# acerbilab/vbmc

Measured on AMD Instinct MI355X. Metric: ELBO+grad evals/sec (Ns=1e4, K=50, D=10, N=400), higher is better.
Workload: dtype f64; 1 GPU; BASELINE configs[2]: D=10 N=400 K=50 Ns=10000/component S=20, R=64 restarts batched per GPU per step, value+gradient, beta=0, no variance; restarts_per_gpu=64, parallelism=one GPU

## Files before the change

### vbmc_amd/csrc/abi_elbo.hip

```cpp
#include <algorithm>
#include <cmath>
#include <mutex>

#include "elbo_kernels.h"
#include "var_kernels.h"
#include "gp_kernels.h"
#include <cstdlib>

extern "C" int vbmc_abi_version(void) { return VBMC_ABI_VERSION; }

static vbmc_status ctx_create_impl(int device, void* stream, vbmc_ctx** out, bool with_aux) {
  if (!out) return VBMC_ERR_INVALID;
  *out = nullptr;
  {
    static std::once_flag hq_once;
    std::call_once(hq_once, [] {
      const char* hq = getenv("VBMC_HW_QUEUES");
      if (!(hq && !strcmp(hq, "0"))) (void)setenv("GPU_MAX_HW_QUEUES", hq && atoi(hq) > 0 ? hq : "8", 0);
    });
  }
  int ndev = 0;
  if (hipGetDeviceCount(&ndev) != hipSuccess || ndev <= 0) return VBMC_ERR_NO_DEVICE;
  if (device < 0 || device >= ndev) return VBMC_ERR_NO_DEVICE;
  hipDeviceProp_t prop;
// ... 846 lines not shown
        const size_t mom_lds = LJ_MFMA_DYN_LDS(DT, nw);
        ElboDims dml = dm;
        dml.S = sh.mode == 1 ? perS : S;
        const double* al = gp->alpha + (size_t)s0 * dm.N;
        const double* gc = gp->gpc + (size_t)s0 * GPC_STRIDE(D);
        if (ns <= 0) {
        } else if (lj_mfma && mom_lds + LJ_MFMA_STATIC_LDS <= 64 * 1024) {
          if (P.compute_grad)
            hipLaunchKernelGGL((k_logjoint_mfma<DT, true>), dim3(ns, R), dim3(WAVE * nw), mom_lds, ls, dml, P.d_vpd,
                               gp->X, gp->d_meanX, al, gc, P.d_delta2, lj_out);
          else
            hipLaunchKernelGGL((k_logjoint_mfma<DT, false>), dim3(ns, R), dim3(WAVE * nw), mom_lds, ls, dml, P.d_vpd,
                               gp->X, gp->d_meanX, al, gc, P.d_delta2, lj_out);
          LAUNCH_CHECK(ctx, "k_logjoint_mfma");
          ctx->last_lj_form = P.compute_grad ? VBMC_LJFORM_MFMA_GRAD : VBMC_LJFORM_MFMA_VALUE;
        } else {
          ctx->last_lj_form = lj_split ? VBMC_LJFORM_VALU_SPLIT : VBMC_LJFORM_VALU_WAVE;
          hipLaunchKernelGGL((k_logjoint<DT>), dim3((K + 3) / 4, ns, R), dim3(lj_split ? WAVE * LJ_MAXW : WAVE), 0, ls, dml, P.d_vpd, gp->X, al, gc,
                             P.d_delta2, lj_out, P.compute_grad);
          LAUNCH_CHECK(ctx, "k_logjoint");
        }
      });
    }
    if (ctx->profiling) HIP_TRY(ctx, hipEventRecord(ctx->ev[1], ls));
    if (sh.mode == 0 && (fork || !P.mc)) hipLaunchKernelGGL(k_lj_reduce, dim3(K, R), dim3(64), 0, ls, S, K, 2 * D + 2, P.d_lj, P.d_ljbar);
    LAUNCH_CHECK(ctx, "k_lj_reduce");
    return VBMC_OK;
  };
  if (fork) {
    HIP_TRY(ctx, hipEventRecord(ctx->ev_fork, st));
    HIP_TRY(ctx, hipStreamWaitEvent(ctx->aux, ctx->ev_fork, 0));
  } else if (sh.mode != 2) {
    vbmc_status s_ = enqueue_logjoint(st);
    if (s_) return s_;
  }
  if (sh.mode == 2) {
    const size_t blk = shard_doubles(P, sh.world), ljn = shard_lj_doubles(P, sh.world);
    const size_t tot = (size_t)R * S * K * (2 * D + 2) + (P.mc ? (size_t)R * K * P.C * P.ncol : 0);
    hipLaunchKernelGGL(k_shard_scatter, dim3((unsigned)std::min<size_t>((tot + 255) / 256, 4096)), dim3(256), 0, st, R, S, K, 2 * D + 2,
                       P.C, P.ncol, sh.world, perS, perC, blk, ljn, sh.gathered, P.d_lj, P.mc ? P.d_part : nullptr);
    LAUNCH_CHECK(ctx, "k_shard_scatter");
    if (!P.mc) hipLaunchKernelGGL(k_lj_reduce, dim3(K, R), dim3(64), 0, st, S, K, 2 * D + 2, P.d_lj, P.d_ljbar);
  }

  FinArgs fa{};
  fa.dm = dm;
  if (P.mc) {
    EntArgs ea{};
    ea.entp = P.d_entp; ea.vpd = P.d_vpd;
    ea.part = sh.mode == 1 ? sh.send + shard_lj_doubles(P, sh.world) : P.d_part;
    ea.D = D; ea.K = K; ea.Mh = P.Mh; ea.C = sh.mode == 1 ? perC : P.C; ea.c0 = c0; ea.tiles_per_chunk = P.tpc; ea.ncol = P.ncol; ea.seed = seed;
    ea.eps = P.d_eps; ea.eps_stride_r = P.eps_stride_r; ea.cutoff = P.cutoff; ea.r0 = P.r0; ea.rstride = P.rstride;
    ea.prio = 1;
    ea.co_c1 = P.co_c1; ea.co_c2 = P.co_c2; ea.co_tpc2 = P.co_tpc2;
    const bool walk = P.walk_tpw > 0;
    if (walk && (sh.mode != 0 || co)) return set_err(ctx, VBMC_ERR_INVALID, "internal: the walking entropy launch was planned for a sharded / role-carrying pass");
    if (walk) { ea.walk_tpw = P.walk_tpw; ea.walk_R = R; }
    int co_rows = 0;
    if (co) {
      LjCo& lc = ea.lj;
      lc.nsplit = lj_co_nsplit(ctx, P);
      lc.nwg = ((K + 3) / 4) * S * lc.nsplit;
      if (P.use_lane) {
        lc.rows = co_rows = 0;
      } else {
        const int gx = P.co_c2 > 0 ? P.co_c1 : nc;
        lc.rows = co_rows = (std::max(lc.nwg, P.co_c2 > 0 ? K * P.co_c2 : 0) + gx - 1) / gx;
      }
      lc.want_grad = P.compute_grad;
      lc.dm = dm; lc.X = gp->X; lc.alpha = gp->alpha; lc.gpc = gp->gpc; lc.delta2 = P.d_delta2; lc.lj = P.d_lj;
    }
    if (ctx->profiling) HIP_TRY(ctx, hipEventRecord(ctx->ev[2], st));
    if (sh.mode != 2 && nc > 0) {
      ctx->last_ent_form = P.use_lane ? VBMC_ENTFORM_LANE : (P.use_mfma ? VBMC_ENTFORM_MFMA : VBMC_ENTFORM_VALU);
      if (co) ctx->last_lj_form = P.use_lane ? VBMC_LJFORM_ROLE_LANE : VBMC_LJFORM_ROLE_MFMA;
    }
    if (sh.mode == 2 || nc <= 0) {
    } else if (P.use_lane) {
      ea.nc_launch = nc;
      int gx = (K * nc + ENT_LANE_WAVES_HOST - 1) / ENT_LANE_WAVES_HOST;
      if (co) gx = std::max(gx, (ea.lj.nwg + ENT_LANE_WAVES_HOST - 1) / ENT_LANE_WAVES_HOST);
      bool ok = launch_entropy_lane(D, K, P.compute_grad != 0, dim3(gx, 1 + co_rows, R), st, ea);
      if (!ok) return set_err(ctx, VBMC_ERR_UNSUPPORTED, "no lane entropy kernel for D = %d, K = %d", D, K);
    } else if (P.use_mfma) {
      bool ok = launch_entropy_mfma(P.qs, P.kt, P.hv, P.compute_grad != 0, walk ? dim3(P.walk_nw, 1, 1) : dim3((co && P.co_c2 > 0) ? P.co_c1 : nc, K + co_rows, R), st, ea);
      if (!ok) return set_err(ctx, VBMC_ERR_UNSUPPORTED, "no MFMA entropy kernel for D = %d", D);
    } else {
      const size_t lds = P.ent_lds;
      DISPATCH_DT(dt, {
        HIP_TRY(ctx, set_entropy_lds<DT>(P.compute_grad != 0, lds));
        launch_entropy<DT>(P.compute_grad != 0, dim3(nc, K, R), lds, st, ea);
      });
    }
    LAUNCH_CHECK(ctx, "the entropy kernel");
    if (ctx->profiling) HIP_TRY(ctx, hipEventRecord(ctx->ev[3], st));
    if (sh.mode == 1) return VBMC_OK;
    if (fork)
      hipLaunchKernelGGL(k_ent_reduce, dim3(K, R), dim3(P.ncol >= 192 ? 256 : (P.ncol >= 96 ? 128 : 64)), 0, st, P.C, P.ncol,
                         P.d_part, P.d_red, P.walk_tpw, (P.Mh + 15) / 16);
    else
      hipLaunchKernelGGL(k_reduce_both, dim3(K, R, 2), dim3(P.ncol >= 192 ? 256 : (P.ncol >= 96 ? 128 : 64)), 0, st, P.C, P.ncol,
                         P.d_part, P.d_red, co ? S * ea.lj.nsplit : S, 2 * D + 2, P.d_lj, P.d_ljbar, P.walk_tpw, (P.Mh + 15) / 16);
    LAUNCH_CHECK(ctx, "k_ent_reduce / k_reduce_both");
    fa.entpart = P.d_red; fa.entlb = nullptr; fa.M = P.Mh; fa.C = 1; fa.ncol = P.ncol;
  } else {
    if (sh.mode == 1) return VBMC_OK;
// ... 723 lines not shown
```

### vbmc_amd/csrc/elbo_types.h

```cpp
#pragma once
#include <hip/hip_runtime.h>

#define WAVE 64

struct VpLayout {
  int D, K;
  __host__ __device__ int mu() const { return 0; }
  __host__ __device__ int sigma() const { return D * K; }
  __host__ __device__ int lambda() const { return D * K + K; }
  __host__ __device__ int w() const { return D * K + K + D; }
  __host__ __device__ int eta() const { return D * K + 2 * K + D; }
  __host__ __device__ int lognf() const { return D * K + 3 * K + D; }
  __host__ __device__ int lnsigma() const { return D * K + 3 * K + D + 1; }
  __host__ __device__ int lnlambda() const { return D * K + 4 * K + D + 1; }
  __host__ __device__ int stride() const { return D * K + 4 * K + 2 * D + 2; }
};
#define ENTP_EXTRA 4
#define GPC_STRIDE(D) (3 * (D) + 2)
#define OUT_HDR 5

struct ElboDims {
  int D, K, R, S, N, T;
  int opt[4];
  int off_mu, off_sigma, off_lambda, off_eta;
};


#define LJ_CO_SPLIT 8
struct LjCo {
  int rows;
  int nwg;
  int nsplit, want_grad;
  ElboDims dm;
  const double *X, *alpha, *gpc, *delta2;
  double* lj;
};

struct EntArgs {
  const double* entp;
  const double* vpd;
  const double* eps;
  long long eps_stride_r;
  double* part;
  int D, K, Mh, C, tiles_per_chunk, ncol;
  int c0;
  int prio;
  unsigned long long seed;
  int r0, rstride;
  double cutoff;
  int nc_launch;
  int co_c1, co_c2, co_tpc2;
  int walk_tpw, walk_R;
  LjCo lj;
};

__host__ __device__ inline int ent_walk_first(long long p, int ntile, int tpw) { return (int)((p * ntile) / tpw); }
__host__ __device__ inline int ent_walk_slots(long long p, int ntile, int tpw) {
  return (int)((p * ntile + ntile - 1) / tpw) - ent_walk_first(p, ntile, tpw) + 1;
}
__host__ __device__ inline int ent_walk_max_slots(int ntile, int tpw) { return (ntile - 1) / tpw + 2; }

#define VB_SMALL_PRIO() __builtin_amdgcn_s_setprio(3)
```

### vbmc_amd/csrc/entropy_mfma.h

```cpp
#pragma once
#include <type_traits>

#include "device_math.h"
#include "elbo_types.h"
#include "exp2_tab1k.h"
#include "logjoint_body.h"

typedef double mf4 __attribute__((ext_vector_type(4)));
struct EntTileAny { static constexpr bool rt = false, val = true; };
struct EntTileFull { static constexpr bool rt = false, val = false; };
struct EntTilePartial { static constexpr bool rt = false, val = true; };
#define VBMC_ENT_SPLIT(KT_, QS_, TL_, HV_) ((HV_) == 1)

#ifdef VBMC_INSTRUMENT
#define VBMC_DBG_WAVES 32768
__device__ unsigned long long g_ent_dbg[6 * VBMC_DBG_WAVES];
#endif

#define VBMC_STAG_FOR(KT_, QS_, TL_) ((KT_) == 1 || (KT_) == 4 || ((KT_) == 2 && (QS_) >= 6) || ((KT_) == 3 && (QS_) <= ((TL_) ? 5 : 8)))



constexpr bool ent_c2_for(int KT, int QS, int TL, int HV) {
  if (HV == 1) {
// ... 9 lines not shown
  }
  if (KT == 2) return !((TL == 1 && QS >= 6) || (TL == 2 && QS >= 5));
  if (KT == 3) return !(TL == 1 && QS == 7);
  return QS != 5;
}
constexpr bool ent_gp2_for(int KT, int QS, int TL, int HV) { return !(HV == 1 && KT == 1 && TL == 0 && QS <= 3); }

template <int HV>
__device__ __forceinline__ void ent_sync() {
  __builtin_amdgcn_fence(__ATOMIC_RELEASE, "wavefront");
  __builtin_amdgcn_wave_barrier();
  __builtin_amdgcn_fence(__ATOMIC_ACQUIRE, "wavefront");
}
template <int HV>
__device__ __forceinline__ void ent_sync_wg() {
  if (HV == 1) ent_sync<1>();
  else __syncthreads();
}

template <int QS, int KT, bool GRAD, bool SPARSE, int HV = 1, int TL = 0, bool CO = false, bool EM = true, bool WALK = false>
#define VBMC_ENT_EO(HV_) true
#define VBMC_ENT_ONE_WAVE(KT_, QS_, TL_, HV_) \
  (((HV_) == 1 && (KT_) == 4 && (QS_) >= 5) || ((HV_) == 1 && (KT_) == 3 && (QS_) >= 8) || ((HV_) == 4 && (KT_) == 4 && (QS_) >= 6) || \
   ((HV_) == 4 && (KT_) == 3 && (QS_) >= 9))
#define VBMC_ENT_WAVES(KT_, QS_, TL_, HV_) \
  (VBMC_ENT_ONE_WAVE(KT_, QS_, TL_, HV_) ? 1 : ((((KT_) <= 2 && (QS_) <= 4) && !((KT_) == 2 && (TL_) == 2 && (HV_) == 1)) ? 3 : 2))
__device__ __forceinline__ void ent_mfma_segment(const EntArgs& a, const int c, const int j, const int r, const int t0, const int t1,
                                                 const int pdone, const int ptot) {
  static_assert(!CO || (HV == 1 && QS <= 8 && !SPARSE), "the log-joint role exists for single-wave dense kernels at D <= 30");
  static_assert(!WALK || (HV == 1 && !CO), "the walk exists for single-wave workgroups without the log-joint role");
  static_assert(KT <= 4 && (HV == 1 || HV == 2 || HV == 4 || HV == 8), "larger mixtures are split over the waves of a workgroup (HV = 2, 4; round 5: 8, K <= 512)");
  static_assert(TL == 0 || ((TL == 1 || TL == 2) && !SPARSE), "the component tail (one or two values per lane) exists for the dense kernels only");
  constexpr int TLN = TL > 0 ? TL : 1;
  constexpr bool SP = SPARSE;
  constexpr int DP = 4 * QS;
  constexpr int NPV = (4 * QS + 15) / 16;
  constexpr int QL = QS;
  __shared__ double Et[16 * DP];
  constexpr bool GP2 = GRAD && ent_gp2_for(KT, QS, TL, HV);
  __shared__ double RQ_all[HV][GP2 ? 32 : 16];
  __shared__ double BND_all[HV][SPARSE ? KT * 16 * 3 : 1];
  constexpr int YXN = NPV * 4 * WAVE;
  constexpr bool EO = VBMC_ENT_EO(HV);
  constexpr bool YXSB = HV > 1 && EO;
  constexpr bool US = EO;
  constexpr bool VBL = GRAD && HV == 1 && (KT >= 3 || NPV >= 2);
  __shared__ double VBS_all[HV][VBL ? KT * 4 * NPV * WAVE : 1];
  constexpr bool C2 = EO && !SPARSE && ent_c2_for(KT, QS, TL, HV);
#define ENT_CI(kt_, rr_) (16 * (kt_) + 4 * (rr_) + lg)
  __shared__ __attribute__((aligned(16))) double SCP_all[HV][C2 ? KT * 16 * 2 : 2];
  __shared__ double BTL_all[HV][TL ? 4 * TL * DP : 1];
  constexpr bool NML = HV > 1 && EO;
  __shared__ double NMS_all[HV][NML ? KT * 4 * WAVE : 1];
#ifdef VBMC_INSTRUMENT
  const unsigned long long wckE = wall_clock64();
#endif
  int tid_ = threadIdx.x;
  if (WALK) asm volatile("" : "+v"(tid_));
  const int tid = tid_, wv = tid >> 6, hv = HV == 1 ? 0 : wv, lane = tid & 63;
  const int li = lane & 15, lg = lane >> 4;
  int D_ = a.D, K_ = a.K;
  const double *entp_ = a.entp, *vpd_ = a.vpd;
  double* part_ = a.part;
  if (WALK) asm volatile("" : "+s"(D_), "+s"(K_), "+s"(entp_), "+s"(vpd_), "+s"(part_));
  const int D = D_, K = K_;
  double* RQ = RQ_all[wv];
  double* NMS = NMS_all[wv];
  double* BND = BND_all[hv];
  double* VBS = VBS_all[hv];
  double* BTL = BTL_all[hv];
  double* SCP = SCP_all[hv];
  const int Kh = (K + HV - 1) / HV;
  const int kbase = hv * Kh;
  const int Kw = min(K, kbase + Kh) - kbase;
  const int PSg = D + ENTP_EXTRA;
  extern __shared__ double PB[];
  double* const TAB = PB;
  double* const YX = PB + VB_EXP_TAB1K_N;
  constexpr int NTH0 = WAVE * HV;
  constexpr int NTB0 = (VB_EXP_TAB1K_N + NTH0 - 1) / NTH0;
  double tt[NTB0];
#pragma unroll
  for (int u = 0; u < NTB0; ++u) tt[u] = c_exp2_tab1k[min(tid + u * NTH0, VB_EXP_TAB1K_N - 1)];
  const double sigj = vpd_[(size_t)r * VpLayout{D, K}.stride() + VpLayout{D, K}.sigma() + j];
  {
    const double* gsrc = entp_ + (size_t)r * K * PSg;
    constexpr int NT = WAVE * HV;
    const int n = K * PSg;
    int idx = tid;
    for (; idx + 7 * NT < n; idx += 8 * NT) {
      double t8[8];
#pragma unroll
      for (int u = 0; u < 8; ++u) t8[u] = gsrc[idx + u * NT];
#pragma unroll
      for (int u = 0; u < 8; ++u) PB[idx + u * NT] = t8[u];
    }
    {
      double t8[8];
#pragma unroll
      for (int u = 0; u < 8; ++u) t8[u] = (idx + u * NT < n) ? gsrc[idx + u * NT] : 0.0;
#pragma unroll
      for (int u = 0; u < 8; ++u) if (idx + u * NT < n) PB[idx + u * NT] = t8[u];
    }
  }
  __syncthreads();
  const double* gp = PB;
  const double* pj = gp + (size_t)j * PSg;
  const double cKj = pj[D + 1];
  const double hj_neg = 0.5 / (sigj * sigj);
  const int nr_last = TL ? 4 : max(1, min(4, (Kw - 16 * (KT - 1) + 3) >> 2));
  constexpr unsigned FULL_MASK = (1u << KT) - 1u;
  const double logwj = SPARSE ? log(pj[D + 2]) : 0.0;

  constexpr double ESC = VB_EXP_TAB1K_SCALE;
  double SA[KT][QL];
  double SC[KT];
  double VB[VBL ? 1 : KT][4][NPV];
  double WF[KT][4];
#pragma unroll
  for (int kt = 0; kt < KT; ++kt) {
    const int k = 16 * kt + li;
    const bool kv = k < Kw;
    const double* pk = gp + (size_t)(kv ? kbase + k : 0) * PSg;
    double h = pk[D];
    double m2 = 0.0;
    for (int d = 0; d < D; ++d) { double t = pk[d] - pj[d]; m2 = fma(t, t, m2); }
    if (SPARSE && lg == 0) {
      BND[(16 * kt + li) * 3 + 0] = sqrt(m2);
      BND[(16 * kt + li) * 3 + 1] = kv ? pk[D + 1] - cKj : -1.0e30;
      BND[(16 * kt + li) * 3 + 2] = h;
    }
#pragma unroll
    for (int q = 0; q < QL; ++q) {
      const int cc = 4 * q + lg;
      if (EO) {
        double sav = (kv && cc < D) ? ESC * (-2.0 * h * (pk[cc] - pj[cc])) : 0.0;
        if (C2) {
          if (cc == D) sav = kv ? ESC * (h + hj_neg) : 0.0;
          if (cc == D + 1) sav = ESC * (kv ? fma(h, m2, pk[D + 1]) - cKj : -1.0e6);
        }
        SA[kt][q] = sav;
      } else {
        double v;
        if (!kv) v = (cc == D + 1) ? -1.0e6 : 0.0;
        else if (cc < D) v = -2.0 * h * (pk[cc] - pj[cc]);
        else if (cc == D) v = h + hj_neg;
        else if (cc == D + 1) v = fma(h, m2, pk[D + 1]) - cKj;
        else v = 0.0;
        SA[kt][q] = ESC * v;
      }
    }
    SC[kt] = ESC * (!kv ? (lg == 1 ? -1.0e6 : 0.0)
                        : (lg == 0 ? h + hj_neg : (lg == 1 ? fma(h, m2, pk[D + 1]) - cKj : 0.0)));
    if (C2 && lg < 2) SCP[(16 * kt + li) * 2 + lg] = 2.0 * SC[kt];
#pragma unroll
    for (int rr = 0; rr < 4; ++rr) {
      const int k2 = ENT_CI(kt, rr);
      const bool kv2 = k2 < Kw;
      const double* p2 = gp + (size_t)(kv2 ? kbase + k2 : 0) * PSg;
      if (GRAD) {
#pragma unroll
        for (int pv = 0; pv < NPV; ++pv) {
          const int col = 16 * pv + li;
          double v = 0.0;
          if (kv2) {
            if (col == 0) v = p2[D + 2];
            else if (col == 1) v = p2[D + 3];
            else if (col < 2 + D) v = p2[D + 3] * (p2[col - 2] - pj[col - 2]);
          }
          if (VBL) VBS[((kt * 4 + rr) * NPV + pv) * WAVE + lane] = v;
          else VB[VBL ? 0 : kt][rr][pv] = v;
        }
      } else {
        WF[kt][rr] = kv2 ? p2[D + 2] : 0.0;
      }
    }
  }

  double tC0[TLN], tC1[TLN], VBt[TLN][NPV], WFt[TLN], Wt[TLN];
#pragma unroll
  for (int u = 0; u < TLN; ++u) {
    tC0[u] = 0.0; tC1[u] = 0.0; WFt[u] = 0.0; Wt[u] = 0.0;
#pragma unroll
    for (int pv = 0; pv < NPV; ++pv) VBt[u][pv] = 0.0;
  }
  if (TL) {
#pragma unroll
    for (int u = 0; u < TLN; ++u) {
      const int tq = 4 * u + lg;
      const int kq = 16 * KT + tq;
      const bool kvq = kq < Kw;
      const double* pq = gp + (size_t)(kvq ? kbase + kq : 0) * PSg;
      const double h = pq[D];
      double m2 = 0.0;
      for (int d = 0; d < D; ++d) { double t = pq[d] - pj[d]; m2 = fma(t, t, m2); }
      tC0[u] = kvq ? ESC * (h + hj_neg) : 0.0;
      tC1[u] = ESC * (kvq ? fma(h, m2, pq[D + 1]) - cKj : -1.0e6);
      for (int d = li; d < DP; d += 16) BTL[tq * DP + d] = (kvq && d < D) ? ESC * (-2.0 * h * (pq[d] - pj[d])) : 0.0;
      if (GRAD) {
#pragma unroll
        for (int pv = 0; pv < NPV; ++pv) {
          const int col = 16 * pv + li;
          double v = 0.0;
          if (kvq) {
            if (col == 0) v = pq[D + 2];
            else if (col == 1) v = pq[D + 3];
            else if (col < 2 + D) v = pq[D + 3] * (pq[col - 2] - pj[col - 2]);
          }
          VBt[u][pv] = v;
        }
      } else {
        WFt[u] = kvq ? pq[D + 2] : 0.0;
      }
    }
  }

  __syncthreads();
  {
#pragma unroll
    for (int u = 0; u < NTB0; ++u) if (VB_EXP_TAB1K_N % NTH0 == 0 || tid + u * NTH0 < VB_EXP_TAB1K_N) TAB[tid + u * NTH0] = tt[u];
  }
  __syncthreads();

#define SAV(kt_, q_) SA[kt_][q_]
  constexpr int VBR = (VBL && NPV == 1 && HV == 1 && KT == 3 && !CO) ? ((EM && QS <= 4) ? (TL == 2 ? 4 : 10) : 12) : 0;
  double VBreg[VBR > 0 ? VBR : 1];
#pragma unroll
  for (int u = 0; u < VBR; ++u) VBreg[u] = VBS[u * WAVE + lane];
#define VBV(kt_, rr_, pv_) (VBL ? (((kt_) * 4 + (rr_)) * NPV + (pv_) < VBR ? VBreg[(((kt_) * 4 + (rr_)) * NPV + (pv_)) < VBR ? (((kt_) * 4 + (rr_)) * NPV + (pv_)) : 0] : VBS[(((kt_) * 4 + (rr_)) * NPV + (pv_)) * WAVE + lane]) : VB[VBL ? 0 : (kt_)][rr_][pv_])
  double accH = 0.0, accG[NPV], accLG[NPV];
  double pm = 1.0;
  int pe = 0, pcnt = 0;
  double Wacc[KT][4];
#pragma unroll
  for (int pv = 0; pv < NPV; ++pv) { accG[pv] = 0.0; accLG[pv] = 0.0; }
#pragma unroll
  for (int kt = 0; kt < KT; ++kt)
#pragma unroll
    for (int rr = 0; rr < 4; ++rr) Wacc[kt][rr] = 0.0;

#ifdef VBMC_INSTRUMENT
  const unsigned long long wck0 = wall_clock64();
#endif
  const int ntile = (a.Mh + 15) >> 4;
  const double sfm0 = lg == 0 ? 1.0 : 0.0, sfm1 = lg == 1 ? 1.0 : 0.0;
  const int emask = (4 * (QS - 1) + lg < D) ? -1 : 0;
  const int emask2 = (QS >= 2 && 4 * (QS - 2) + lg < D) ? -1 : 0;
  const double* epsr = a.eps ? a.eps + (size_t)r * a.eps_stride_r + (size_t)j * a.Mh * D : nullptr;
  constexpr bool EPF = EM && HV == 1 && QS <= 4 && KT <= 3 && !SPARSE;
  double epre[EPF ? QS : 1];
  auto eps_fetch = [&](const int tile) {
#pragma unroll
    for (int u = 0; u < (EPF ? QS : 0); ++u) {
      const int idx = lane + u * WAVE, i = idx / DP, d = idx - i * DP;
      double v = 0.0;
      if (tile < t1 && d < D && tile * 16 + i < a.Mh) v = epsr[(size_t)(tile * 16 + i) * D + d];
      epre[u] = v;
    }
  };
  if (EPF && epsr) eps_fetch(t0);
  if (!epsr && (HV == 1 || hv == 0))
    for (int idx = lane; idx < 16 * DP; idx += WAVE) Et[idx] = 0.0;
  const int evm1 = emask, evm2 = emask2;
  const double c2u1 = (4 * (QS - 1) + lg == D) ? 1.0 : 0.0, c2o1 = (4 * (QS - 1) + lg == D + 1) ? 1.0 : 0.0;
  const double c2u2 = (QS >= 2 && 4 * (QS - 2) + lg == D) ? 1.0 : 0.0;

  auto tile_body = [&](const int tile, auto pkind) __attribute__((always_inline)) {
    using PK = decltype(pkind);
    const int b0 = tile * 16;
    ent_sync_wg<HV>();
    if (HV > 1 && hv != 0) {
    } else if (EPF && epsr) {
#pragma unroll
      for (int u = 0; u < (EPF ? QS : 0); ++u) Et[lane + u * WAVE] = US ? sigj * epre[u] : epre[u];
      eps_fetch(tile + 1);
    } else if (epsr) {
      for (int idx = lane; idx < 16 * DP; idx += WAVE) {
        const int i = idx / DP, d = idx - i * DP;
        Et[idx] = (d < D && b0 + i < a.Mh) ? (US ? sigj * epsr[(size_t)(b0 + i) * D + d] : epsr[(size_t)(b0 + i) * D + d]) : 0.0;
      }
    } else {
      unsigned long long seed_t = a.seed;
      if (WALK) asm volatile("" : "+s"(seed_t));
#pragma unroll
      for (int q = lg; q < QS; q += 4) {
        double z4[4] = {0.0, 0.0, 0.0, 0.0};
#define VBMC_RNG_CALL_FOR(KT_, QS_, TL_, HV_) ((HV_) == 2 && (((KT_) == 2 && (TL_) == 2 && (QS_) == 5) || ((KT_) == 3 && (TL_) == 0 && (QS_) == 7)))
        if constexpr (!VBMC_RNG_CALL_FOR(KT, QS, TL, HV)) {
        if (q < (D + 3) / 4) { const vb_d4 zz = vb_normal4i(seed_t, (unsigned)(b0 + li), (unsigned)j, (unsigned)(a.r0 + r * a.rstride), (unsigned)q); z4[0] = zz[0]; z4[1] = zz[1]; z4[2] = zz[2]; z4[3] = zz[3]; }
        } else {
        if (q < (D + 3) / 4) vb_normal4(seed_t, (unsigned)(b0 + li), (unsigned)j, (unsigned)(a.r0 + r * a.rstride), (unsigned)q, z4);
        }
#undef VBMC_RNG_CALL_FOR
        if (q < (D + 3) / 4) {
#pragma unroll
        for (int t = 0; t < 4; ++t) Et[li * DP + 4 * q + t] = US ? sigj * z4[t] : z4[t];
        }
      }
    }
    ent_sync_wg<HV>();
    double ev[QS];
    double e2 = 0.0;
#pragma unroll
    for (int q = 0; q < QS; ++q) {
      ev[q] = Et[li * DP + 4 * q + lg];
      if (q == QS - 1) ev[q] = __hiloint2double(__double2hiint(ev[q]) & evm1, __double2loint(ev[q]) & evm1);
      if (QS >= 2 && q == QS - 2) ev[q] = __hiloint2double(__double2hiint(ev[q]) & evm2, __double2loint(ev[q]) & evm2);
      e2 = fma(ev[q], ev[q], e2);
    }
    e2 = xor_sum16(e2);
    e2 = xor_sum32(e2);
    double shift = US ? fma(-e2, hj_neg, cKj) : cKj - 0.5 * e2;
    const double u2 = US ? e2 : sigj * sigj * e2;
    if (US && SPARSE) e2 *= 2.0 * hj_neg;
    constexpr bool partial = PK::val;
    const bool svalid = b0 + li < a.Mh;
    if (partial) shift = svalid ? shift : 0.0;
    unsigned act = FULL_MASK;
    if (SPARSE) {
      double e2m = e2;
      e2m = fmax(e2m, __shfl_xor(e2m, 1, 64)); e2m = fmax(e2m, __shfl_xor(e2m, 2, 64));
      e2m = fmax(e2m, __shfl_xor(e2m, 4, 64)); e2m = fmax(e2m, __shfl_xor(e2m, 8, 64));
      const double umax = sigj * sqrt(e2m);
      const double own = 0.5 * e2m - logwj;
      act = 0u;
#pragma unroll
      for (int kt = 0; kt < KT; ++kt) {
        const double* bk = BND + (16 * kt + li) * 3;
        const double t = fmax(0.0, bk[0] - umax);
        const double bnd = fma(bk[2] * t, t, bk[1]) + own;
        if (__any(bnd > -a.cutoff)) act |= 1u << kt;
      }
    }

    mf4 n[KT], nm[(EO && !NML) ? KT : 1];
    if (EO) {
      const double sfc = fma(u2, sfm0, sfm1);
      double sfl[QL];
#pragma unroll
      for (int q = 0; q < QL; ++q) sfl[q] = US ? ev[q] : ev[q] * sigj;
      if (C2) {
        sfl[QL - 1] = fma(u2, c2u1, sfl[QL - 1] + c2o1);
        if (QS >= 2) sfl[QL >= 2 ? QL - 2 : 0] = fma(u2, c2u2, sfl[QL >= 2 ? QL - 2 : 0]);
      }
#pragma unroll
      for (int kt = 0; kt < KT; ++kt) {
        n[kt] = (mf4){0.0, 0.0, 0.0, 0.0};
        if (!NML) nm[(EO && !NML) ? kt : 0] = (mf4){0.0, 0.0, 0.0, 0.0};
        if (C2) {
#pragma unroll
          for (int q = 0; q < QL; ++q) n[kt] = __builtin_amdgcn_mfma_f64_16x16x4f64(SAV(kt, q), sfl[q], n[kt], 0, 0, 0);
          mf4 e2nd;
#pragma unroll
          for (int rr = 0; rr < 4; ++rr) {
            const double2 pr = *reinterpret_cast<const double2*>(SCP + ENT_CI(kt, rr) * 2);
            e2nd[rr] = fma(pr.x, u2, pr.y) - n[kt][rr];
          }
          if (NML) {
#pragma unroll
            for (int rr = 0; rr < 4; ++rr) NMS[(kt * 4 + rr) * WAVE + lane] = e2nd[rr];
          } else {
            nm[(EO && !NML) ? kt : 0] = e2nd;
          }
        } else
        if (!SP || ((act >> kt) & 1u)) {
          const mf4 cacc = __builtin_amdgcn_mfma_f64_16x16x4f64(SC[kt], sfc, n[kt], 0, 0, 0);
          n[kt] = cacc;
#pragma unroll
          for (int q = 0; q < QL; ++q)
            n[kt] = __builtin_amdgcn_mfma_f64_16x16x4f64(SAV(kt, q), sfl[q], n[kt], 0, 0, 0);
          if (NML) {
            const mf4 e2nd = 2.0 * cacc - n[kt];
#pragma unroll
            for (int rr = 0; rr < 4; ++rr) NMS[(kt * 4 + rr) * WAVE + lane] = e2nd[rr];
          } else {
            nm[(EO && !NML) ? kt : 0] = 2.0 * cacc - n[kt];
          }
        }
      }
    }

    double ntl[TLN], ntm[TLN];
#pragma unroll
    for (int u = 0; u < TLN; ++u) { ntl[u] = 0.0; ntm[u] = 0.0; }
    if (TL) {
#pragma unroll
      for (int u = 0; u < TLN; ++u) {
        double lt = 0.0;
#pragma unroll
        for (int d = 0; d < DP; ++d) lt = fma(BTL[(4 * u + lg) * DP + d], Et[li * DP + d], lt);
        if (!US) lt *= sigj;
        const double ct = fma(tC0[u], u2, tC1[u]);
        ntl[u] = ct + lt;
        ntm[u] = ct - lt;
      }
    }

    auto exps = [&](mf4 (&x)[KT], auto k0c, auto k1c) {
      constexpr int k0 = decltype(k0c)::value, k1 = decltype(k1c)::value;
#pragma unroll
      for (int kt = k0; kt < k1; ++kt) {
        if (kt < KT - 1) {
          if (!SP || ((act >> kt) & 1u)) x[kt] = vb_exp_tab1k4<VB_EXP_TAB1K_QUAD>(x[kt], TAB);
          else x[kt] = (mf4){0.0, 0.0, 0.0, 0.0};
        } else if (SP && !((act >> (KT - 1)) & 1u)) {
          x[KT - 1] = (mf4){0.0, 0.0, 0.0, 0.0};
        } else if (nr_last == 4) {
          x[KT - 1] = vb_exp_tab1k4<VB_EXP_TAB1K_QUAD>(x[KT - 1], TAB);
        } else {
          mf4 t = x[KT - 1];
          x[KT - 1] = (mf4){0.0, 0.0, 0.0, 0.0};
          x[KT - 1][0] = vb_exp_tab1k<VB_EXP_TAB1K_QUAD>(t[0], TAB);
          if (nr_last > 1) x[KT - 1][1] = vb_exp_tab1k<VB_EXP_TAB1K_QUAD>(t[1], TAB);
          if (nr_last > 2) x[KT - 1][2] = vb_exp_tab1k<VB_EXP_TAB1K_QUAD>(t[2], TAB);
        }
      }
    };
    auto texp = [&](double (&t)[TLN]) {
      if (TL) {
#pragma unroll
        for (int u = 0; u < TLN; ++u) t[u] = vb_exp_tab1k<VB_EXP_TAB1K_QUAD>(t[u], TAB);
      }
    };
    auto pvstep = [&](mf4 (&x)[KT], mf4 (&Y)[NPV], int sg, const double (&tn)[TLN]) {
      constexpr bool TWO = NPV == 1 && KT <= 2;
      mf4 Y2s[TWO ? NPV : 1];
      mf4 (&Y2)[TWO ? NPV : 1] = Y2s;
#pragma unroll
      for (int pv = 0; pv < NPV; ++pv) { Y[pv] = (mf4){0.0, 0.0, 0.0, 0.0}; if (TWO) Y2[pv] = (mf4){0.0, 0.0, 0.0, 0.0}; }
#pragma unroll
      for (int kt = 0; kt < KT - 1; ++kt) {
        if (SP && !((act >> kt) & 1u)) continue;
#pragma unroll
        for (int pv = 0; pv < NPV; ++pv) {
          mf4& Yb = TWO ? Y2[TWO ? pv : 0] : Y[pv];
          Y[pv] = __builtin_amdgcn_mfma_f64_16x16x4f64(x[kt][0], VBV(kt, 0, pv), Y[pv], 0, 0, 0);
          Yb = __builtin_amdgcn_mfma_f64_16x16x4f64(x[kt][1], VBV(kt, 1, pv), Yb, 0, 0, 0);
          Y[pv] = __builtin_amdgcn_mfma_f64_16x16x4f64(x[kt][2], VBV(kt, 2, pv), Y[pv], 0, 0, 0);
          Yb = __builtin_amdgcn_mfma_f64_16x16x4f64(x[kt][3], VBV(kt, 3, pv), Yb, 0, 0, 0);
        }
      }
#pragma unroll
      for (int pv = 0; pv < NPV; ++pv) {
        mf4& Yb = TWO ? Y2[TWO ? pv : 0] : Y[pv];
        if (SP && !((act >> (KT - 1)) & 1u)) { if (TWO) Y[pv] += Yb; continue; }
        Y[pv] = __builtin_amdgcn_mfma_f64_16x16x4f64(x[KT - 1][0], VBV(KT - 1, 0, pv), Y[pv], 0, 0, 0);
        if (nr_last > 1) Yb = __builtin_amdgcn_mfma_f64_16x16x4f64(x[KT - 1][1], VBV(KT - 1, 1, pv), Yb, 0, 0, 0);
        if (nr_last > 2) Y[pv] = __builtin_amdgcn_mfma_f64_16x16x4f64(x[KT - 1][2], VBV(KT - 1, 2, pv), Y[pv], 0, 0, 0);
        if (nr_last > 3) Yb = __builtin_amdgcn_mfma_f64_16x16x4f64(x[KT - 1][3], VBV(KT - 1, 3, pv), Yb, 0, 0, 0);
        if (TL) {
#pragma unroll
          for (int u = 0; u < TLN; ++u) Y[pv] = __builtin_amdgcn_mfma_f64_16x16x4f64(tn[u], VBt[u][pv], Y[pv], 0, 0, 0);
        }
        if (TWO) Y[pv] += Yb;
      }
      if (HV > 1) {
        if (YXSB && sg == 1) __syncthreads();
#pragma unroll
        for (int pv = 0; pv < NPV; ++pv)
#pragma unroll
          for (int rr = 0; rr < 4; ++rr) YX[((YXSB ? 0 : sg) * HV + hv) * YXN + (pv * 4 + rr) * WAVE + lane] = Y[pv][rr];
        __syncthreads();
#pragma unroll
        for (int pv = 0; pv < NPV; ++pv)
#pragma unroll
          for (int rr = 0; rr < 4; ++rr) {
            double t = YX[((YXSB ? 0 : sg) * HV + 0) * YXN + (pv * 4 + rr) * WAVE + lane];
#pragma unroll
            for (int w = 1; w < HV; ++w) t += YX[((YXSB ? 0 : sg) * HV + w) * YXN + (pv * 4 + rr) * WAVE + lane];
            Y[pv][rr] = t;
          }
      }
    };
    auto put_q = [&](mf4 (&Y)[NPV]) {
      if (GP2 ? li < 2 : li == 0) {
#pragma unroll
        for (int rr = 0; rr < 4; ++rr) RQ[(GP2 ? 16 * li : 0) + lg + 4 * rr] = Y[0][rr];
      }
      ent_sync<HV>();
    };
    double arq = 0.0;
    constexpr bool TQ = GP2 && US && NPV == 1 && HV == 1 && EO && KT == 3 && QS <= 3 && !CO && !EM && VBMC_STAG_FOR(KT, QS, TL);
    double tq[TQ ? 4 : 1];
    auto get_rq = [&]() -> double {
      double qs_ = RQ[li];
      double rqs = vb_rcp(qs_);
      if (partial) {
        qs_ = svalid ? qs_ : 1.0;
        rqs = svalid ? rqs : 0.0;
      }
      if (GP2) arq = RQ[GP2 ? 16 + li : 0] * rqs;
      pm *= __builtin_amdgcn_frexp_mant(qs_);
      pe += __builtin_amdgcn_frexp_exp(qs_);
      accH += shift;
      return rqs;
    };
    auto wacc = [&](mf4 (&x)[KT], double rqs, const double (&tn)[TLN]) {
      if (TL) {
#pragma unroll
        for (int u = 0; u < TLN; ++u) Wt[u] = fma(tn[u], rqs, Wt[u]);
      }
#pragma unroll
      for (int kt = 0; kt < KT; ++kt) {
        if (SP && !((act >> kt) & 1u)) continue;
#pragma unroll
        for (int rr = 0; rr < 4; ++rr) Wacc[kt][rr] = fma(x[kt][rr], rqs, Wacc[kt][rr]);
      }
    };
    auto put_rq = [&](double rqs) {
      ent_sync<HV>();
      if (lg == 0) { RQ[li] = rqs; if (GP2) RQ[GP2 ? 16 + li : 0] = arq; }
      ent_sync<HV>();
    };
    auto gradpieces = [&](mf4 (&Y)[NPV], double ssig, auto sgc) {
      constexpr int SG = decltype(sgc)::value;
      if constexpr (GP2) {
#pragma unroll
        for (int rr = 0; rr < 4; ++rr) {
          const int i = lg + 4 * rr;
          const double rq = RQ[i], ar = RQ[GP2 ? 16 + i : 0];
#pragma unroll
          for (int pv = 0; pv < NPV; ++pv) {
            if (HV > 1 && (pv % HV) != hv) continue;
            const int d = min(max(16 * pv + li - 2, 0), DP - 1);
            double tv;
            if (TQ) { if (SG >= 0) tq[TQ ? rr : 0] = Et[i * DP + d]; tv = tq[TQ ? rr : 0]; }
            else tv = Et[i * DP + d];
            const double t = (US && SG > 0) ? tv : ((US && SG < 0) ? -tv : ssig * tv);
            const double gd = fma(t, ar, -(Y[pv][rr] * rq));
            accG[pv] += gd;
            accLG[pv] = fma(t, gd, accLG[pv]);
          }
        }
        ent_sync<HV>();
        return;
      }
      const int base = lane & 48;
#pragma unroll
      for (int rr = 0; rr < 4; ++rr) {
        const int i = lg + 4 * rr;
        const double Av = __shfl(Y[0][rr], base | 1, 64);
        const double rq = RQ[i];
#pragma unroll
        for (int pv = 0; pv < NPV; ++pv) {
          if (HV > 1 && (pv % HV) != hv) continue;
          const int d = 16 * pv + li - 2;
          if (d >= 0 && d < D) {
            const double t = (US && SG > 0) ? Et[i * DP + d] : ((US && SG < 0) ? -Et[i * DP + d] : ssig * Et[i * DP + d]);
            const double gd = (t * Av - Y[pv][rr]) * rq;
            accG[pv] += gd;
            accLG[pv] = fma(t, gd, accLG[pv]);
          }
        }
      }
      ent_sync<HV>();
    };
    auto fold = [&]() {
// ... 53 lines not shown
        if (GRAD) {
          mf4 Y[NPV];
          pvstep(n, Y, sg, ntl);
          put_q(Y);
          const double rqs = get_rq();
          wacc(n, rqs, ntl);
          put_rq(rqs);
          gradpieces(Y, ssig, std::integral_constant<int, 0>{});
        } else {
          double qp = 0.0;
#pragma unroll
          for (int kt = 0; kt < KT; ++kt)
#pragma unroll
            for (int rr = 0; rr < 4; ++rr) qp = fma(WF[kt][rr], n[kt][rr], qp);
          if (TL) {
#pragma unroll
            for (int u = 0; u < TLN; ++u) qp = fma(WFt[u], ntl[u], qp);
          }
          qp += __shfl_xor(qp, 16, 64);
          qp += __shfl_xor(qp, 32, 64);
          if (HV > 1) {
            if (YXSB && sg == 1) __syncthreads();
            YX[((YXSB ? 0 : sg) * HV + hv) * YXN + lane] = qp;
            __syncthreads();
            qp = YX[((YXSB ? 0 : sg) * HV + 0) * YXN + lane];
#pragma unroll
            for (int w = 1; w < HV; ++w) qp += YX[((YXSB ? 0 : sg) * HV + w) * YXN + lane];
          }
          double qs_ = qp;
          if (partial) qs_ = svalid ? qp : 1.0;
          pm *= __builtin_amdgcn_frexp_mant(qs_);
          pe += __builtin_amdgcn_frexp_exp(qs_);
          accH += shift;
        }
        fold();
        if (sg) break;
        sg = 1;
        ssig = US ? -1.0 : -sigj;
        if (EO) {
#pragma unroll
          for (int kt = 0; kt < KT; ++kt) {
            if (NML) {
#pragma unroll
              for (int rr = 0; rr < 4; ++rr) n[kt][rr] = NMS[(kt * 4 + rr) * WAVE + lane];
            } else {
              n[kt] = nm[(EO && !NML) ? kt : 0];
            }
          }
        }
#pragma unroll
        for (int u = 0; u < TLN; ++u) ntl[u] = ntm[u];
      }
    }
  };
  if constexpr (VBMC_ENT_SPLIT(KT, QS, TL, HV)) {
    const int tf = min(t1, a.Mh >> 4);
    constexpr bool PRIO = CO ? QS <= 4 : VBMC_ENT_WAVES(KT, QS, TL, HV) > 1;
    const bool pr = PRIO && a.prio != 0;
    const int q1 = pr ? t0 + (ptot + 3) / 4 - pdone : -1, q2 = pr ? t0 + (ptot + 1) / 2 - pdone : -1, q3 = pr ? t0 + (3 * ptot + 3) / 4 - pdone : -1;
    if (pr && pdone == 0) __builtin_amdgcn_s_setprio(3);
    for (int tile = t0; tile < tf; ++tile) {
      if (tile == q1) __builtin_amdgcn_s_setprio(2);
      if (tile == q2) __builtin_amdgcn_s_setprio(1);
      if (tile == q3) __builtin_amdgcn_s_setprio(0);
      tile_body(tile, EntTileFull{});
    }
    if (tf < t1) tile_body(tf, EntTilePartial{});
  } else {
    for (int tile = t0; tile < t1; ++tile) tile_body(tile, EntTileAny{});
  }
#ifdef VBMC_INSTRUMENT
  const unsigned long long wck1 = wall_clock64();
#endif
  if (WALK) accH += vb_log_pos(pm, &pe) + 0.693147180559945309417 * (double)pe;
  else accH += log(pm) + 0.693147180559945309417 * (double)pe;
  if (lg != 0) accH = 0.0;

  double* o = part_ + (((size_t)r * K + j) * a.C + c) * a.ncol;
  accH = wave_sum(accH);
  if (lane == 0 && hv == 0) o[0] = accH;
  if (GRAD) {
    double sgsum = 0.0;
#pragma unroll
    for (int pv = 0; pv < NPV; ++pv) {
      double g = accG[pv], lgd = accLG[pv] / sigj;
      g += __shfl_xor(g, 16, 64); g += __shfl_xor(g, 32, 64);
      lgd += __shfl_xor(lgd, 16, 64); lgd += __shfl_xor(lgd, 32, 64);
      const int d = 16 * pv + li - 2;
      const bool dv = d >= 0 && d < D;
      const bool mine = HV == 1 || (pv % HV) == hv;
      if (dv && lg == 0 && mine) { o[1 + d] = g; o[2 + D + d] = lgd; }
      sgsum += (dv && lg == 0 && mine) ? lgd : 0.0;
    }
    sgsum = wave_sum(sgsum);
    if (HV > 1) {
      __syncthreads();
      if (lane == 0) YX[hv * YXN] = sgsum;
      __syncthreads();
      sgsum = YX[0];
#pragma unroll
      for (int w = 1; w < HV; ++w) sgsum += YX[w * YXN];
    }
    if (lane == 0 && hv == 0) o[1 + D] = sgsum;
#pragma unroll
    for (int kt = 0; kt < KT; ++kt)
#pragma unroll
      for (int rr = 0; rr < 4; ++rr) {
        double wv = Wacc[kt][rr];
        wv += __shfl_xor(wv, 1, 64); wv += __shfl_xor(wv, 2, 64);
        wv += __shfl_xor(wv, 4, 64); wv += __shfl_xor(wv, 8, 64);
        const int k = ENT_CI(kt, rr);
        if (li == 0 && k < Kw) o[2 + 2 * D + kbase + k] = wv;
      }
    if (TL) {
#pragma unroll
      for (int u = 0; u < TLN; ++u) {
        double wv = Wt[u];
        wv += __shfl_xor(wv, 1, 64); wv += __shfl_xor(wv, 2, 64);
        wv += __shfl_xor(wv, 4, 64); wv += __shfl_xor(wv, 8, 64);
        const int k = 16 * KT + 4 * u + lg;
        if (li == 0 && k < Kw) o[2 + 2 * D + kbase + k] = wv;
      }
    }
  }
#ifdef VBMC_INSTRUMENT
  if (lane == 0) {
    const size_t w = ((size_t)r * K + j) * a.C + c;
    if (w < VBMC_DBG_WAVES) {
      g_ent_dbg[6 * w + 0] = wckE; g_ent_dbg[6 * w + 1] = wck0; g_ent_dbg[6 * w + 2] = wck1; g_ent_dbg[6 * w + 3] = wall_clock64();
      g_ent_dbg[6 * w + 4] = __builtin_amdgcn_s_getreg(63492);
      g_ent_dbg[6 * w + 5] = __builtin_amdgcn_s_getreg(63508);
    }
  }
#endif
#undef VBV
#undef SAV
#undef ENT_CI
}

template <int QS, int KT, bool GRAD, bool SPARSE, int HV = 1, int TL = 0, bool CO = false, bool EM = true, bool WALK = false>
__global__ void __launch_bounds__(WAVE * HV, CO ? (QS <= 4 ? 2 : 1) : VBMC_ENT_WAVES(KT, QS, TL, HV)) k_entropy_mfma(EntArgs a) {
  const int ntile = (a.Mh + 15) >> 4;
  constexpr bool walk = WALK;
  int c = (int)blockIdx.x, j = CO ? (int)blockIdx.y - a.lj.rows : (int)blockIdx.y, r = (int)blockIdx.z;
  int tlo = ((int)blockIdx.x + a.c0) * a.tiles_per_chunk, thi = min(tlo + a.tiles_per_chunk, ntile), pdone = 0, rem = 0;
  if (!WALK && a.co_c2 > 0 && c >= a.co_c1) {
    tlo = a.co_c1 * a.tiles_per_chunk + (c - a.co_c1) * a.co_tpc2;
    thi = min(tlo + a.co_tpc2, ntile);
  }
  if (CO) {
    if ((int)blockIdx.y < a.lj.rows) {
      extern __shared__ double PB[];
      lj_co_role<4 * QS>(a.lj, a.vpd, PB);
      const int e = (int)(blockIdx.y * gridDim.x + blockIdx.x);
      if (a.co_c2 <= 0 || e >= a.K * a.co_c2) return;
      j = e / a.co_c2;
      c = a.co_c1 + (e - j * a.co_c2);
      tlo = a.co_c1 * a.tiles_per_chunk + (c - a.co_c1) * a.co_tpc2;
      thi = min(tlo + a.co_tpc2, ntile);
      __syncthreads();
    }
  }
  if (walk) {
    const int g = (int)blockIdx.x * a.walk_tpw;
    rem = min(a.walk_tpw, a.K * a.walk_R * ntile - g);
    const int p = g / ntile;
    tlo = g - p * ntile;
    r = p / a.K;
    j = p - r * a.K;
    c = (int)blockIdx.x - (g - tlo) / a.walk_tpw;
  }
  const int ptot = walk ? rem : thi - tlo;
  for (;;) {
    if (walk) thi = min(ntile, tlo + rem);
    ent_mfma_segment<QS, KT, GRAD, SPARSE, HV, TL, CO, EM, WALK>(a, c, j, r, tlo, thi, pdone, ptot);
    if (!walk) break;
    pdone += thi - tlo;
    rem -= thi - tlo;
    if (rem <= 0) break;
    if (++j == a.K) { j = 0; ++r; }
    tlo = 0;
    c = 0;
    __syncthreads();
  }
}
```

Before: 29820 evals/s.

## Prune negligible mixture components per tile in MFMA entropy kernel

Adds a per-wave pruning path to the entropy kernel. Components are sorted in shared memory by a proximity key to the current component, and per-tile distance bounds skip the exp and MFMA work for component groups whose contribution falls below a cutoff (default 40 in log space, overridable by an env var). The path is enabled only when at most 16 components can matter, and gradient outputs are written back through the permutation. In exchange it adds a sort, extra syncs and per-tile ballots, and it introduces a bounded approximation error for the skipped terms.

```diff
diff --git a/vbmc_amd/csrc/abi_elbo.hip b/vbmc_amd/csrc/abi_elbo.hip
--- a/vbmc_amd/csrc/abi_elbo.hip
+++ b/vbmc_amd/csrc/abi_elbo.hip
@@ -922,6 +922,8 @@
     ea.D = D; ea.K = K; ea.Mh = P.Mh; ea.C = sh.mode == 1 ? perC : P.C; ea.c0 = c0; ea.tiles_per_chunk = P.tpc; ea.ncol = P.ncol; ea.seed = seed;
     ea.eps = P.d_eps; ea.eps_stride_r = P.eps_stride_r; ea.cutoff = P.cutoff; ea.r0 = P.r0; ea.rstride = P.rstride;
     ea.prio = 1;
+    static const double prune_cut = [] { const char* e = getenv("VBMC_ENT_PRUNE"); if (!e) return 40.0; const double v = atof(e); return v > 0.0 ? v : 0.0; }();
+    ea.prune = prune_cut;
     ea.co_c1 = P.co_c1; ea.co_c2 = P.co_c2; ea.co_tpc2 = P.co_tpc2;
     const bool walk = P.walk_tpw > 0;
     if (walk && (sh.mode != 0 || co)) return set_err(ctx, VBMC_ERR_INVALID, "internal: the walking entropy launch was planned for a sharded / role-carrying pass");
diff --git a/vbmc_amd/csrc/elbo_types.h b/vbmc_amd/csrc/elbo_types.h
--- a/vbmc_amd/csrc/elbo_types.h
+++ b/vbmc_amd/csrc/elbo_types.h
@@ -48,6 +48,7 @@
   unsigned long long seed;
   int r0, rstride;
   double cutoff;
+  double prune;
   int nc_launch;
   int co_c1, co_c2, co_tpc2;
   int walk_tpw, walk_R;
diff --git a/vbmc_amd/csrc/entropy_mfma.h b/vbmc_amd/csrc/entropy_mfma.h
--- a/vbmc_amd/csrc/entropy_mfma.h
+++ b/vbmc_amd/csrc/entropy_mfma.h
@@ -85,6 +85,10 @@
   __shared__ double BTL_all[HV][TL ? 4 * TL * DP : 1];
   constexpr bool NML = HV > 1 && EO;
   __shared__ double NMS_all[HV][NML ? KT * 4 * WAVE : 1];
+  constexpr bool PRN = HV == 1 && !SPARSE && KT >= 3;
+  __shared__ int PERM[PRN ? WAVE : 1];
+  __shared__ double PKEY[PRN ? WAVE : 1];
+  __shared__ double PBND[PRN ? 3 * WAVE : 1];
 #ifdef VBMC_INSTRUMENT
   const unsigned long long wckE = wall_clock64();
 #endif
@@ -143,7 +147,42 @@
   const double hj_neg = 0.5 / (sigj * sigj);
   const int nr_last = TL ? 4 : max(1, min(4, (Kw - 16 * (KT - 1) + 3) >> 2));
   constexpr unsigned FULL_MASK = (1u << KT) - 1u;
-  const double logwj = SPARSE ? log(pj[D + 2]) : 0.0;
+  const double logwj = (SPARSE || PRN) ? log(pj[D + 2]) : 0.0;
+  double pcut = PRN ? a.prune : 0.0;
+  if (WALK) asm volatile("" : "+s"(pcut));
+  bool pon = PRN && pcut > 0.0;
+  if (PRN) {
+    const int k = lane;
+    const bool kv = k < Kw;
+    const double* pk = gp + (size_t)(kv ? k : 0) * PSg;
+    double m2 = 0.0;
+    for (int d = 0; d < D; ++d) { double t = pk[d] - pj[d]; m2 = fma(t, t, m2); }
+    {
+      const double ut2 = sigj * sigj * (D + 4.0 * sqrt(2.0 * D));
+      const double t = fmax(0.0, sqrt(m2) - sqrt(ut2));
+      const double b = fma(pk[D] * t, t, pk[D + 1] - cKj) + fma(ut2, hj_neg, -logwj);
+      const unsigned long long need = __ballot(kv && !(b <= -pcut));
+      pon = pon && __popcll(need) <= 16;
+    }
+    double key = k == j ? __builtin_inf() : fma(pk[D], m2, pk[D + 1]);
+    if (!(key == key)) key = -__builtin_inf();
+    PKEY[k] = key;
+    ent_sync<1>();
+    int rk = k;
+    if (pon && kv) {
+      rk = 0;
+      for (int l = 0; l < Kw; ++l) {
+        const double o = PKEY[l];
+        rk += (o > key || (o == key && l < k)) ? 1 : 0;
+      }
+    }
+    PERM[rk] = k;
+    PBND[3 * rk + 0] = sqrt(m2);
+    PBND[3 * rk + 1] = kv ? pk[D + 1] - cKj : -1.0e300;
+    PBND[3 * rk + 2] = pk[D];
+    ent_sync<1>();
+  }
+#define ENT_PK(s_) (PRN ? PERM[(s_)] : (s_))
 
   constexpr double ESC = VB_EXP_TAB1K_SCALE;
   double SA[KT][QL];
@@ -154,7 +193,7 @@
   for (int kt = 0; kt < KT; ++kt) {
     const int k = 16 * kt + li;
     const bool kv = k < Kw;
-    const double* pk = gp + (size_t)(kv ? kbase + k : 0) * PSg;
+    const double* pk = gp + (size_t)(kv ? kbase + ENT_PK(k) : 0) * PSg;
     double h = pk[D];
     double m2 = 0.0;
     for (int d = 0; d < D; ++d) { double t = pk[d] - pj[d]; m2 = fma(t, t, m2); }
@@ -190,7 +229,7 @@
     for (int rr = 0; rr < 4; ++rr) {
       const int k2 = ENT_CI(kt, rr);
       const bool kv2 = k2 < Kw;
-      const double* p2 = gp + (size_t)(kv2 ? kbase + k2 : 0) * PSg;
+      const double* p2 = gp + (size_t)(kv2 ? kbase + ENT_PK(k2) : 0) * PSg;
       if (GRAD) {
 #pragma unroll
         for (int pv = 0; pv < NPV; ++pv) {
@@ -223,7 +262,7 @@
       const int tq = 4 * u + lg;
       const int kq = 16 * KT + tq;
       const bool kvq = kq < Kw;
-      const double* pq = gp + (size_t)(kvq ? kbase + kq : 0) * PSg;
+      const double* pq = gp + (size_t)(kvq ? kbase + ENT_PK(kq) : 0) * PSg;
       const double h = pq[D];
       double m2 = 0.0;
       for (int d = 0; d < D; ++d) { double t = pq[d] - pj[d]; m2 = fma(t, t, m2); }
@@ -298,8 +337,9 @@
   const double c2u1 = (4 * (QS - 1) + lg == D) ? 1.0 : 0.0, c2o1 = (4 * (QS - 1) + lg == D + 1) ? 1.0 : 0.0;
   const double c2u2 = (QS >= 2 && 4 * (QS - 2) + lg == D) ? 1.0 : 0.0;
 
-  auto tile_body = [&](const int tile, auto pkind) __attribute__((always_inline)) {
+  auto tile_body = [&](const int tile, auto pkind, auto prc) __attribute__((always_inline)) {
     using PK = decltype(pkind);
+    constexpr bool PRT = PRN && decltype(prc)::value;
     const int b0 = tile * 16;
     ent_sync_wg<HV>();
     if (HV > 1 && hv != 0) {
@@ -365,6 +405,20 @@
         if (__any(bnd > -a.cutoff)) act |= 1u << kt;
       }
     }
+    int ng = 1 << 20;
+    if (PRT && pon) {
+      double e2m = e2;
+      e2m = fmax(e2m, __shfl_xor(e2m, 1, 64)); e2m = fmax(e2m, __shfl_xor(e2m, 2, 64));
+      e2m = fmax(e2m, __shfl_xor(e2m, 4, 64)); e2m = fmax(e2m, __shfl_xor(e2m, 8, 64));
+      const double umax = sqrt(e2m);
+      const double own = fma(e2m, hj_neg, -logwj);
+      const double t = fmax(0.0, PBND[3 * lane] - umax);
+      const double bnd = fma(PBND[3 * lane + 2] * t, t, PBND[3 * lane + 1]) + own;
+      const unsigned long long m = __ballot(!(bnd <= -pcut));
+      ng = m ? (67 - __builtin_clzll(m)) >> 2 : 1 << 20;
+    }
+#define ENT_KON(kt_) (!PRT || ng > 4 * (kt_))
+#define ENT_RON(rr_) (!PRT || ng > (rr_))
 
     mf4 n[KT], nm[(EO && !NML) ? KT : 1];
     if (EO) {
@@ -380,7 +434,8 @@
       for (int kt = 0; kt < KT; ++kt) {
         n[kt] = (mf4){0.0, 0.0, 0.0, 0.0};
         if (!NML) nm[(EO && !NML) ? kt : 0] = (mf4){0.0, 0.0, 0.0, 0.0};
-        if (C2) {
+        if (kt > 0 && !ENT_KON(kt)) {
+        } else if (C2) {
 #pragma unroll
           for (int q = 0; q < QL; ++q) n[kt] = __builtin_amdgcn_mfma_f64_16x16x4f64(SAV(kt, q), sfl[q], n[kt], 0, 0, 0);
           mf4 e2nd;
@@ -416,7 +471,7 @@
     double ntl[TLN], ntm[TLN];
 #pragma unroll
     for (int u = 0; u < TLN; ++u) { ntl[u] = 0.0; ntm[u] = 0.0; }
-    if (TL) {
+    if (TL && ENT_KON(KT)) {
 #pragma unroll
       for (int u = 0; u < TLN; ++u) {
         double lt = 0.0;
@@ -433,7 +488,13 @@
       constexpr int k0 = decltype(k0c)::value, k1 = decltype(k1c)::value;
 #pragma unroll
       for (int kt = k0; kt < k1; ++kt) {
-        if (kt < KT - 1) {
+        if (PRT && kt == 0 && (KT > 1 || nr_last == 4)) {
+          x[0][0] = vb_exp_tab1k<VB_EXP_TAB1K_QUAD>(x[0][0], TAB);
+#pragma unroll
+          for (int rr = 1; rr < 4; ++rr) x[0][rr] = ENT_RON(rr) ? vb_exp_tab1k<VB_EXP_TAB1K_QUAD>(x[0][rr], TAB) : 0.0;
+        } else if (PRT && !ENT_KON(kt)) {
+          x[kt] = (mf4){0.0, 0.0, 0.0, 0.0};
+        } else if (kt < KT - 1) {
           if (!SP || ((act >> kt) & 1u)) x[kt] = vb_exp_tab1k4<VB_EXP_TAB1K_QUAD>(x[kt], TAB);
           else x[kt] = (mf4){0.0, 0.0, 0.0, 0.0};
         } else if (SP && !((act >> (KT - 1)) & 1u)) {
@@ -450,7 +511,7 @@
       }
     };
     auto texp = [&](double (&t)[TLN]) {
-      if (TL) {
+      if (TL && ENT_KON(KT)) {
 #pragma unroll
         for (int u = 0; u < TLN; ++u) t[u] = vb_exp_tab1k<VB_EXP_TAB1K_QUAD>(t[u], TAB);
       }
@@ -464,24 +525,26 @@
 #pragma unroll
       for (int kt = 0; kt < KT - 1; ++kt) {
         if (SP && !((act >> kt) & 1u)) continue;
+        if (PRT && kt > 0 && !ENT_KON(kt)) continue;
 #pragma unroll
         for (int pv = 0; pv < NPV; ++pv) {
           mf4& Yb = TWO ? Y2[TWO ? pv : 0] : Y[pv];
           Y[pv] = __builtin_amdgcn_mfma_f64_16x16x4f64(x[kt][0], VBV(kt, 0, pv), Y[pv], 0, 0, 0);
-          Yb = __builtin_amdgcn_mfma_f64_16x16x4f64(x[kt][1], VBV(kt, 1, pv), Yb, 0, 0, 0);
-          Y[pv] = __builtin_amdgcn_mfma_f64_16x16x4f64(x[kt][2], VBV(kt, 2, pv), Y[pv], 0, 0, 0);
-          Yb = __builtin_amdgcn_mfma_f64_16x16x4f64(x[kt][3], VBV(kt, 3, pv), Yb, 0, 0, 0);
+          if (kt > 0 || ENT_RON(1)) Yb = __builtin_amdgcn_mfma_f64_16x16x4f64(x[kt][1], VBV(kt, 1, pv), Yb, 0, 0, 0);
+          if (kt > 0 || ENT_RON(2)) Y[pv] = __builtin_amdgcn_mfma_f64_16x16x4f64(x[kt][2], VBV(kt, 2, pv), Y[pv], 0, 0, 0);
+          if (kt > 0 || ENT_RON(3)) Yb = __builtin_amdgcn_mfma_f64_16x16x4f64(x[kt][3], VBV(kt, 3, pv), Yb, 0, 0, 0);
         }
       }
 #pragma unroll
       for (int pv = 0; pv < NPV; ++pv) {
         mf4& Yb = TWO ? Y2[TWO ? pv : 0] : Y[pv];
         if (SP && !((act >> (KT - 1)) & 1u)) { if (TWO) Y[pv] += Yb; continue; }
+        if (PRT && !ENT_KON(KT - 1)) { if (TWO) Y[pv] += Yb; continue; }
         Y[pv] = __builtin_amdgcn_mfma_f64_16x16x4f64(x[KT - 1][0], VBV(KT - 1, 0, pv), Y[pv], 0, 0, 0);
-        if (nr_last > 1) Yb = __builtin_amdgcn_mfma_f64_16x16x4f64(x[KT - 1][1], VBV(KT - 1, 1, pv), Yb, 0, 0, 0);
-        if (nr_last > 2) Y[pv] = __builtin_amdgcn_mfma_f64_16x16x4f64(x[KT - 1][2], VBV(KT - 1, 2, pv), Y[pv], 0, 0, 0);
-        if (nr_last > 3) Yb = __builtin_amdgcn_mfma_f64_16x16x4f64(x[KT - 1][3], VBV(KT - 1, 3, pv), Yb, 0, 0, 0);
-        if (TL) {
+        if (nr_last > 1 && (KT > 1 || ENT_RON(1))) Yb = __builtin_amdgcn_mfma_f64_16x16x4f64(x[KT - 1][1], VBV(KT - 1, 1, pv), Yb, 0, 0, 0);
+        if (nr_last > 2 && (KT > 1 || ENT_RON(2))) Y[pv] = __builtin_amdgcn_mfma_f64_16x16x4f64(x[KT - 1][2], VBV(KT - 1, 2, pv), Y[pv], 0, 0, 0);
+        if (nr_last > 3 && (KT > 1 || ENT_RON(3))) Yb = __builtin_amdgcn_mfma_f64_16x16x4f64(x[KT - 1][3], VBV(KT - 1, 3, pv), Yb, 0, 0, 0);
+        if (TL && ENT_KON(KT)) {
 #pragma unroll
           for (int u = 0; u < TLN; ++u) Y[pv] = __builtin_amdgcn_mfma_f64_16x16x4f64(tn[u], VBt[u][pv], Y[pv], 0, 0, 0);
         }
@@ -529,13 +592,14 @@
       return rqs;
     };
     auto wacc = [&](mf4 (&x)[KT], double rqs, const double (&tn)[TLN]) {
-      if (TL) {
+      if (TL && ENT_KON(KT)) {
 #pragma unroll
         for (int u = 0; u < TLN; ++u) Wt[u] = fma(tn[u], rqs, Wt[u]);
       }
 #pragma unroll
       for (int kt = 0; kt < KT; ++kt) {
         if (SP && !((act >> kt) & 1u)) continue;
+        if (PRT && kt > 0 && !ENT_KON(kt)) continue;
 #pragma unroll
         for (int rr = 0; rr < 4; ++rr) Wacc[kt][rr] = fma(x[kt][rr], rqs, Wacc[kt][rr]);
       }
@@ -695,7 +759,10 @@
         for (int u = 0; u < TLN; ++u) ntl[u] = ntm[u];
       }
     }
+#undef ENT_KON
+#undef ENT_RON
   };
+  auto tiles = [&](auto prc) __attribute__((always_inline)) {
   if constexpr (VBMC_ENT_SPLIT(KT, QS, TL, HV)) {
     const int tf = min(t1, a.Mh >> 4);
     constexpr bool PRIO = CO ? QS <= 4 : VBMC_ENT_WAVES(KT, QS, TL, HV) > 1;
@@ -706,11 +773,20 @@
       if (tile == q1) __builtin_amdgcn_s_setprio(2);
       if (tile == q2) __builtin_amdgcn_s_setprio(1);
       if (tile == q3) __builtin_amdgcn_s_setprio(0);
-      tile_body(tile, EntTileFull{});
-    }
-    if (tf < t1) tile_body(tf, EntTilePartial{});
+      tile_body(tile, EntTileFull{}, prc);
+    }
+    if (tf < t1) tile_body(tf, EntTilePartial{}, prc);
   } else {
-    for (int tile = t0; tile < t1; ++tile) tile_body(tile, EntTileAny{});
+    for (int tile = t0; tile < t1; ++tile) tile_body(tile, EntTileAny{}, prc);
+  }
+  };
+  if constexpr (PRN && WALK) {
+    tiles(std::true_type{});
+  } else if constexpr (PRN) {
+    if (pon) tiles(std::true_type{});
+    else tiles(std::false_type{});
+  } else {
+    tiles(std::false_type{});
   }
 #ifdef VBMC_INSTRUMENT
   const unsigned long long wck1 = wall_clock64();
@@ -753,7 +829,7 @@
         wv += __shfl_xor(wv, 1, 64); wv += __shfl_xor(wv, 2, 64);
         wv += __shfl_xor(wv, 4, 64); wv += __shfl_xor(wv, 8, 64);
         const int k = ENT_CI(kt, rr);
-        if (li == 0 && k < Kw) o[2 + 2 * D + kbase + k] = wv;
+        if (li == 0 && k < Kw) o[2 + 2 * D + kbase + ENT_PK(k)] = wv;
       }
     if (TL) {
 #pragma unroll
@@ -762,7 +838,7 @@
         wv += __shfl_xor(wv, 1, 64); wv += __shfl_xor(wv, 2, 64);
         wv += __shfl_xor(wv, 4, 64); wv += __shfl_xor(wv, 8, 64);
         const int k = 16 * KT + 4 * u + lg;
-        if (li == 0 && k < Kw) o[2 + 2 * D + kbase + k] = wv;
+        if (li == 0 && k < Kw) o[2 + 2 * D + kbase + ENT_PK(k)] = wv;
       }
     }
   }
@@ -779,6 +855,7 @@
 #undef VBV
 #undef SAV
 #undef ENT_CI
+#undef ENT_PK
 }
 
 template <int QS, int KT, bool GRAD, bool SPARSE, int HV = 1, int TL = 0, bool CO = false, bool EM = true, bool WALK = false>
```

After: 50740 evals/s, median of 6. 70.1% higher.
